# Eclectic-Sheep/sheeprl

Measured on NVIDIA H100. Metric: Dreamer-V3 train-steps/sec (S, bs16 seq64 horizon15, 64x64x3 obs), higher is better.
Workload: dtype f32

## Files before the change

sheeprl_b200/csrc/rssm_scan.cu:

```cuda
#include "b200rl.h"
#include "common.cuh"

namespace {

constexpr int SCAN_G = 128;
constexpr int SCAN_NT = 512;
constexpr int SCAN_NW = SCAN_NT / 32;
constexpr int MAXB = 16;
constexpr int MAXRPU = 8;
constexpr int KS_MAX = 8;
constexpr int CLS_SLICES = 8;

typedef unsigned long long u64;

__host__ __device__ inline int r4(int x) { return (x + 3) / 4 * 4; }
__host__ __device__ inline int imax(int a, int b) { return a > b ? a : b; }
__host__ __device__ inline int imin(int a, int b) { return a < b ? a : b; }

__host__ __device__ inline int owned_groups(int width, int cta) {
  const int groups = (width + 3) / 4;
  return (groups > cta) ? (groups - cta + SCAN_G - 1) / SCAN_G : 0;
}
__host__ __device__ inline int owned_cols(int width, int cta) {
  int n = 0;
  for (int gi = cta; gi * 4 < width; gi += SCAN_G) n += (width - gi * 4 < 4) ? width - gi * 4 : 4;
  return n;
}

struct Workspace {
  int* error;
  long long* prof;
  u64* ll;
  int* zidx;
  float* ln_stats;
};

struct LLGeo {
  size_t z, x, sx, s, h, r, a, b, c, d, sb, sc, sd, total;
};

__host__ __device__ inline LLGeo make_ll(int S, int Dx, int R, int Dr, int Z) {
  LLGeo g;
  size_t o = 0;
  g.z = o; o += 2 * (size_t)MAXB * S;
  g.x = o; o += 2 * (size_t)MAXB * Dx;
  g.sx = o; o += 2 * (size_t)MAXB * SCAN_G * 2;
  g.s = o; o += 2 * (size_t)MAXB * SCAN_G * 2;
  g.h = o; o += 2 * (size_t)MAXB * R;
  g.r = o; o += 2 * (size_t)MAXB * Dr;
  g.a = o; o += 2 * (size_t)MAXB * Z;
  g.b = o; o += 2 * (size_t)MAXB * Dr;
  g.c = o; o += 2 * (size_t)MAXB * 3 * R;
  g.d = o; o += 2 * (size_t)MAXB * Dx;
  g.sb = o; o += 2 * (size_t)MAXB * SCAN_G * 2;
  g.sc = o; o += 2 * (size_t)MAXB * SCAN_G * 2;
  g.sd = o; o += 2 * (size_t)MAXB * SCAN_G * 2;
  g.total = o;
  return g;
}

constexpr size_t WS_HEADER = 256, WS_PROF = 2 * 32 * sizeof(long long);

__host__ __device__ inline size_t ws_ll_bytes(int S, int D, int Dx, int R, int Dr) {
  return make_ll(S, Dx, R, Dr, S * D).total * sizeof(u64);
}
__host__ __device__ inline size_t ws_bytes(int T, int B, int S, int D, int Dx, int R, int Dr) {
  return WS_HEADER + WS_PROF + ws_ll_bytes(S, D, Dx, R, Dr) + sizeof(int) * (size_t)T * B * S +
         sizeof(float) * 3 * (size_t)T * B * 2 + 256;
}
// ... 33 lines not shown
  bool dead;
  __device__ __forceinline__ void init(int* e) { error = e; polls = 0; t0 = 0; dead = false; }
  __device__ __forceinline__ bool fail() {
    if (dead) return true;
    if ((++polls & 255u) == 0u) {
      if (t0 == 0) t0 = clock64();
      if (clock64() - t0 > 4000000000LL) { atomicExch(error, 1); dead = true; }
      else if (*(volatile int*)error != 0) dead = true;
    }
    return dead;
  }
};

__device__ __forceinline__ float ll_wait(const u64* p, unsigned tag, Spin& sp) {
  u64 v = ll_load(p);
  while ((unsigned)(v >> 32) != tag) {
    if (sp.fail()) break;
    v = ll_load(p);
  }
  return __uint_as_float((unsigned)v);
}

template <int LL_UNROLL>
__device__ __noinline__ void ll_recv(float* dst, int ds, const u64* src, int ss, int rows, int n, unsigned tag, int tid, Spin& sp) {
  const int half = n >> 1;
  int rg = 0, kp = tid, nrg = 1, kstep = SCAN_NT;
  if (half < SCAN_NT) { rg = tid / half; kp = tid - rg * half; nrg = SCAN_NT / half; kstep = half; if (rg >= nrg) return; }
  for (int k = 2 * kp; k < n; k += 2 * kstep) {
    for (int r0 = rg; r0 < rows; r0 += nrg * LL_UNROLL) {
      u64 a[LL_UNROLL], b[LL_UNROLL];
#pragma unroll
      for (int u = 0; u < LL_UNROLL; ++u)
        if (r0 + u * nrg < rows) ll_load2(src + (size_t)(r0 + u * nrg) * ss + k, a[u], b[u]);
      for (;;) {
        bool stale = false;
#pragma unroll
        for (int u = 0; u < LL_UNROLL; ++u)
          if (r0 + u * nrg < rows && ((unsigned)(a[u] >> 32) != tag || (unsigned)(b[u] >> 32) != tag)) stale = true;
        if (!stale || sp.fail()) break;
#pragma unroll
        for (int u = 0; u < LL_UNROLL; ++u)
          if (r0 + u * nrg < rows && ((unsigned)(a[u] >> 32) != tag || (unsigned)(b[u] >> 32) != tag))
            ll_load2(src + (size_t)(r0 + u * nrg) * ss + k, a[u], b[u]);
      }
#pragma unroll
      for (int u = 0; u < LL_UNROLL; ++u)
        if (r0 + u * nrg < rows)
          *reinterpret_cast<float2*>(dst + (r0 + u * nrg) * ds + k) =
              make_float2(__uint_as_float((unsigned)a[u]), __uint_as_float((unsigned)b[u]));
    }
  }
}

struct Slot {
  int b, cj, col;
  bool ok;
};
__device__ __forceinline__ Slot make_slot(int e, int per_row, int B, int cta, int width) {
  Slot s;
  s.b = per_row > 0 ? e / per_row : 0;
  s.cj = e - s.b * per_row;
  s.col = (cta + (s.cj >> 2) * SCAN_G) * 4 + (s.cj & 3);
  s.ok = per_row > 0 && s.b < B && s.col < width;
  return s;
}

__device__ __forceinline__ float fsilu(float x) { return __fdividef(x, 1.f + __expf(-x)); }

__device__ __forceinline__ void mma_tf32(float (&d)[4], const unsigned (&a)[4], unsigned b0, unsigned b1) {
  asm volatile("mma.sync.aligned.m16n8k8.row.col.f32.tf32.tf32.f32 {%0,%1,%2,%3}, {%4,%5,%6,%7}, {%8,%9}, {%0,%1,%2,%3};"
               : "+f"(d[0]), "+f"(d[1]), "+f"(d[2]), "+f"(d[3])
               : "r"(a[0]), "r"(a[1]), "r"(a[2]), "r"(a[3]), "r"(b0), "r"(b1));
}
__device__ __forceinline__ unsigned tf32_hi(float x) { return __float_as_uint(x) & 0xffffe000u; }
// ... 24 lines not shown
    }
    {
      const unsigned ah[4] = {tf32_hi(va.z), tf32_hi(vb.z), tf32_hi(va.w), tf32_hi(vb.w)};
      const unsigned al[4] = {tf32_lo(va.z), tf32_lo(vb.z), tf32_lo(va.w), tf32_lo(vb.w)};
      const unsigned bh0 = tf32_hi(vw.z), bh1 = tf32_hi(vw.w), bl0 = tf32_lo(vw.z), bl1 = tf32_lo(vw.w);
      mma_tf32(dx, ah, bl0, bl1);
      mma_tf32(dy, al, bh0, bh1);
      mma_tf32(d, ah, bh0, bh1);
    }
  }
#pragma unroll
  for (int i = 0; i < 4; ++i) d[i] += dx[i] + dy[i];
  const int c = 2 * t;
  if (c < nvalid) {
    part[(size_t)g * ldp + c0 + c] = d[0];
    part[(size_t)(g + 8) * ldp + c0 + c] = d[2];
  }
  if (c + 1 < nvalid) {
    part[(size_t)g * ldp + c0 + c + 1] = d[1];
    part[(size_t)(g + 8) * ldp + c0 + c + 1] = d[3];
  }
}

__device__ __noinline__ int product(const float* X, int xs, const float* wbase, int wst, int ngroups, int K, int B,
                                       float* PART, int ldp, int cbase, int tid) {
  if (ngroups <= 0) return 0;
  const int lane = tid & 31, wid = tid >> 5;
  const int ncols = ngroups * 4, ntiles = (ncols + 7) >> 3, Kp = r4(K);
  int ks = imin(KS_MAX, imax(1, SCAN_NW / ntiles));
  const int kchunk = ((Kp + ks - 1) / ks + 15) / 16 * 16;
  ks = (Kp + kchunk - 1) / kchunk;
  for (int item = wid; item < ntiles * ks; item += SCAN_NW) {
    const int sl = item / ntiles, tile = item - sl * ntiles;
    const int k0 = sl * kchunk, k1 = imin(Kp, k0 + kchunk);
    mma_item(X, xs, B, wbase + (size_t)tile * 8 * wst, wst, imin(8, ncols - tile * 8), k0, k1,
             PART + (size_t)sl * MAXB * ldp, ldp, cbase + tile * 8, lane);
  }
  return ks;
}

__device__ __forceinline__ float part_sum(const float* PART, int ldp, int ks, int b, int c) {
  float v = 0.f;
  for (int s = 0; s < ks; ++s) v += PART[((size_t)s * MAXB + b) * ldp + c];
  return v;
}

__device__ __noinline__ void class_product(const float* X, int xs, const float* W, int wst, int D, int Kp, int nr, float* PART,
                                              int tid) {
  const int lane = tid & 31, wid = tid >> 5, g = lane >> 2, t = lane & 3;
  const int sl = wid % CLS_SLICES, half = wid / CLS_SLICES;
  const int kc = ((Kp + CLS_SLICES - 1) / CLS_SLICES + 15) / 16 * 16;
  const int k0 = sl * kc, k1 = imin(Kp, k0 + kc);
  const int n0 = half * 16;
  if (n0 >= D) return;
  const bool r_ok = g < nr, n_ok0 = n0 + g < D, n_ok1 = n0 + 8 + g < D;
  const float* xa = X + (size_t)g * xs;
  const float* w0 = W + (size_t)(n0 + g) * wst;
  const float* w1 = W + (size_t)(n0 + 8 + g) * wst;
  float d0[4] = {0.f, 0.f, 0.f, 0.f}, d1[4] = {0.f, 0.f, 0.f, 0.f};
  float e0[4] = {0.f, 0.f, 0.f, 0.f}, e1[4] = {0.f, 0.f, 0.f, 0.f};
  for (int kb = k0; kb < k1; kb += 16) {
    const int k = kb + 4 * t;
    const bool k_ok = k < k1;
    float4 va = make_float4(0.f, 0.f, 0.f, 0.f), v0 = va, v1 = va;
    if (r_ok && k_ok) va = *reinterpret_cast<const float4*>(xa + k);
    if (n_ok0 && k_ok) v0 = *reinterpret_cast<const float4*>(w0 + k);
    if (n_ok1 && k_ok) v1 = *reinterpret_cast<const float4*>(w1 + k);
    {
      const unsigned ah[4] = {tf32_hi(va.x), 0u, tf32_hi(va.y), 0u}, al[4] = {tf32_lo(va.x), 0u, tf32_lo(va.y), 0u};
      mma_tf32(e0, ah, tf32_lo(v0.x), tf32_lo(v0.y)); mma_tf32(e1, ah, tf32_lo(v1.x), tf32_lo(v1.y));
// ... 94 lines not shown
  const int S = FIX ? 32 : a.S, D = FIX ? 32 : a.D, Z = S * D, R = FIX ? 512 : a.R, Dx = FIX ? 512 : a.Dx, Dr = FIX ? 512 : a.Dr;
  const int NB = T * B;
  const GeoF g = make_geo_f(Dims{B, S, D, R, Dx, Dr, a.A}, cta);
  const Workspace ws = carve(a.workspace, T, B, S, D, Dx, R, Dr);
  const LLGeo L = make_ll(S, Dx, R, Dr, Z);
  float* Wg = sm + g.oWg;
  float* Wr1 = sm + g.oWr1;
  float* W2 = sm + g.oW2;
  float* Xh = sm + g.oXh;
  float* Xx = sm + g.oXx;
  float* PART = sm + g.oPart;
  float* ACC = sm + g.oAcc;
  float* Win = sm + g.oWin;
  float* X0 = sm + g.oX0;
  float* H0 = sm + g.oPar;
  float* LNXG = H0 + g.sR;
  float* LNXB = LNXG + g.sDx;
  float* LNRG = LNXB + g.sDx;
  float* LNRB = LNRG + g.sDr;
  float* misc = sm + g.oMisc;
  int* z0idx = (int*)(sm + g.oInt);
  int* zall = z0idx + 64;
  int* nctab = zall + MAXB * 64;
  int* nxtab = nctab + SCAN_G;
  const int ldp = g.ldp, xxs = imax(g.sDx, g.sDr);
  const bool sampler = g.unit_g >= 0;
  __shared__ long long sprof[32];
  const bool prof_on = (cta < 2) && tid == 0;
  long long* prof = sprof;
  if (tid < 32) sprof[tid] = 0;
  long long tlast = prof_on ? clock64() : 0;
  Spin sp;
  sp.init(ws.error);

  for (int e = tid; e < g.total; e += SCAN_NT) sm[e] = 0.f;
  __syncthreads();
  for (int gi = 0; gi < g.ngh; ++gi)
    for (int part = 0; part < 3; ++part) {
      float* dst = Wg + (size_t)(gi * 3 + part) * 4 * g.wgst;
      const float* Wp = a.W_g + (size_t)part * R * (R + Dx);
      load_rows4(dst, g.wgst, 0, Wp, R + Dx, (cta + gi * SCAN_G) * 4, R, 0, R, g.sR, tid);
      load_rows4(dst, g.wgst, g.sR, Wp, R + Dx, (cta + gi * SCAN_G) * 4, R, R, Dx, g.sDx, tid);
    }
  for (int gi = 0; gi < g.ngr; ++gi)
    load_rows4(Wr1 + (size_t)gi * 4 * g.sR, g.sR, 0, a.W_r1, a.ld_wr1, (cta + gi * SCAN_G) * 4, Dr, 0, R, g.sR, tid);
  if (sampler)
    for (int e = tid; e < D * Dr; e += SCAN_NT) {
      const int d = e / Dr, k = e - d * Dr;
      W2[d * g.w2st + k] = a.W_r2[((size_t)g.unit_g * D + d) * Dr + k];
    }
  for (int k = tid; k < R; k += SCAN_NT) H0[k] = a.h0[k];
  for (int k = tid; k < Dx; k += SCAN_NT) { LNXG[k] = a.lnx_g[k]; LNXB[k] = a.lnx_b[k]; }
  for (int k = tid; k < Dr; k += SCAN_NT) { LNRG[k] = a.lnr_g[k]; LNRB[k] = a.lnr_b[k]; }
  for (int c = tid; c < SCAN_G; c += SCAN_NT) { nctab[c] = owned_cols(R, c); nxtab[c] = owned_cols(Dx, c); }
  for (int gi = 0; gi < g.ngx; ++gi)
    load_rows4(Win + (size_t)gi * 4 * g.kin, g.kin, 0, a.W_in, Z + A, (cta + gi * SCAN_G) * 4, Dx, 0, Z + A, g.kin, tid);
  if (wid == 0) {
    for (int gq = 0; gq < S; ++gq) {
      int best = 0;
      for (int d = lane; d < D; d += 32)
        if (a.z0[gq * D + d] > 0.5f) best = d;
#pragma unroll
      for (int o = 16; o > 0; o >>= 1) best = max(best, __shfl_xor_sync(0xffffffffu, best, o));
      if (lane == 0) z0idx[gq] = best;
    }
  }
  __syncthreads();
  for (int cj = tid; cj < g.ngx * 4; cj += SCAN_NT) {
    float acc = 0.f;
    for (int gq = 0; gq < S; ++gq) acc += Win[(size_t)cj * g.kin + gq * D + z0idx[gq]];
    X0[cj] = acc;
  }
  if (sampler)
    for (int e = tid; e < g.unit_nr * D; e += SCAN_NT) {
      const int b = g.unit_r0 + e / D, d = e % D;
      a.z_in[(size_t)b * Z + g.unit_g * D + d] = a.first[b] * ((z0idx[g.unit_g] == d) ? 1.f : 0.f);
    }
  const int nh4 = g.ngh * 4, nh12 = g.ngh * 12, nr4 = g.ngr * 4, nx4 = g.ngx * 4;
  const Slot sH = make_slot(tid, nh4, B, cta, R);
  const Slot sX = make_slot(tid, nx4, B, cta, Dx);
  const int nxcol = owned_cols(Dx, cta);
  const Slot sR_ = make_slot(tid, nr4, B, cta, Dr);
  const int pb = nh12 > 0 ? tid / nh12 : 0, pc = tid - pb * nh12;
  const int pcol = (cta + (pc / 12) * SCAN_G) * 4 + (pc & 3), ppart = (pc % 12) >> 2;
  const bool pok = nh12 > 0 && pb < B && pcol < R;
  float lg_g[3] = {0.f, 0.f, 0.f}, lg_b[3] = {0.f, 0.f, 0.f};
  if (sH.ok)
#pragma unroll
    for (int part = 0; part < 3; ++part) { lg_g[part] = a.lng_g[part * R + sH.col]; lg_b[part] = a.lng_b[part * R + sH.col]; }
  const int ncol3 = 3 * owned_cols(R, cta);
  const float bias2 = (sampler && lane < D) ? a.b_r2[g.unit_g * D + lane] : 0.f;
  float first_next = (tid < B) ? a.first[tid] : 0.f;
  __syncthreads();
  prof_mark(prof, 0, tlast, prof_on);

  for (int t = 0; t < T; ++t) {
    const size_t row0 = (size_t)t * B;
    const int par = t & 1;
    const unsigned tag = (unsigned)t + 1u;
    if (tid < MAXB) misc[tid] = first_next;
    if (tid < MAXB) first_next = (tid < B && t + 1 < T) ? a.first[row0 + B + tid] : 0.f;
    const float pe_pref = sR_.ok ? a.pe[(row0 + sR_.b) * Dr + sR_.col] : 0.f;
    float noise_pref = 1.f, fnext = 0.f;
    if (sampler && wid < g.unit_nr) {
      if (lane < D) noise_pref = a.noise[(row0 + g.unit_r0 + wid) * Z + (size_t)g.unit_g * D + lane];
      if (t + 1 < T) fnext = a.first[row0 + B + g.unit_r0 + wid];
    }
    __syncthreads();
    const float* fl = misc;

    if (t > 0)
      for (int e = tid; e < B * S; e += SCAN_NT) {
        const int b = e / S, gq = e - b * S;
        zall[b * 64 + gq] = (int)__float_as_uint(ll_wait(ws.ll + L.z + ((size_t)(par ^ 1) * MAXB + b) * S + gq, (unsigned)t, sp));
      }
    __syncthreads();
    prof_mark(prof, 2, tlast, prof_on);
    for (int b = wid; b < B; b += SCAN_NW) {
      const float f = fl[b];
      float rowv[4] = {0.f, 0.f, 0.f, 0.f};
      float rs = 0.f;
      int rcnt = 0;
      for (int c0 = 0; c0 < nx4; c0 += 4) {
        const int cj = c0 + (lane >> 3), part = lane & 7;
        const int col = (cta + (cj >> 2) * SCAN_G) * 4 + (cj & 3);
        const bool okc = cj < nx4 && col < Dx;
        float acc = 0.f;
        if (okc && t > 0 && f != 1.f) {
          const float* wrow = Win + (size_t)cj * g.kin;
          const int gper = (S + 7) >> 3, g_lo = part * gper, g_hi = imin(S, g_lo + gper);
          for (int gq = g_lo; gq < g_hi; ++gq) acc += wrow[gq * D + zall[b * 64 + gq]];
        }
        acc += __shfl_xor_sync(0xffffffffu, acc, 4);
        acc += __shfl_xor_sync(0xffffffffu, acc, 2);
        acc += __shfl_xor_sync(0xffffffffu, acc, 1);
        if (okc && part == 0) {
          float aa = 0.f;
          for (int qq = 0; qq < A; ++qq) aa = fmaf(a.actions[(row0 + b) * A + qq], Win[(size_t)cj * g.kin + Z + qq], aa);
          const float xv = (1.f - f) * (acc + aa) + f * X0[cj];
          ll_store(ws.ll + L.x + ((size_t)par * MAXB + b) * Dx + col, xv, tag);
          a.x_pre[(row0 + b) * Dx + col] = xv;
          rowv[c0 >> 2] = xv;
          rs += xv;
          ++rcnt;
        }
      }
      rs = warp_sum(rs);
      const float mean = nxcol > 0 ? rs / (float)nxcol : 0.f;
      float m2 = 0.f;
      for (int i = 0; i < 4; ++i)
        if (i < rcnt) { const float d = rowv[i] - mean; m2 = fmaf(d, d, m2); }
      m2 = warp_sum(m2);
      if (lane == 0) ll_store2(ws.ll + L.sx + (((size_t)par * MAXB + b) * SCAN_G + cta) * 2, mean, m2, tag);
    }
    if (cta == (t % SCAN_G))
      for (int e = tid; e < B * A; e += SCAN_NT) a.a_in[row0 * A + e] = (1.f - fl[e / A]) * a.actions[row0 * A + e];
    prof_mark(prof, 3, tlast, prof_on);

    for (int b = 0; b < B; ++b) {
      const float f = fl[b];
      if (f != 0.f || t == 0)
        for (int k = tid; k < R; k += SCAN_NT) Xh[b * g.sR + k] = (1.f - f) * ((t > 0) ? Xh[b * g.sR + k] : 0.f) + f * H0[k];
    }
    __syncthreads();
    prof_mark(prof, 12, tlast, prof_on);
    const int ksh = product(Xh, g.sR, Wg, g.wgst, g.ngh * 3, R, B, PART, ldp, 0, tid);
    prof_mark(prof, 1, tlast, prof_on);
    __syncthreads();
    const float acch = pok ? part_sum(PART, ldp, ksh, pb, pc) : 0.f;
    const float hin = sH.ok ? Xh[sH.b * g.sR + sH.col] : 0.f;
    prof_mark(prof, 13, tlast, prof_on);

    ll_recv<8>(Xx, xxs, ws.ll + L.x + (size_t)par * MAXB * Dx, Dx, B, Dx, tag, tid, sp);
    for (int b = wid; b < B; b += SCAN_NW) {
      float pm[SCAN_G / 32], pq[SCAN_G / 32];
      u64 x[SCAN_G / 32], y[SCAN_G / 32];
#pragma unroll
      for (int i = 0; i < SCAN_G / 32; ++i)
        ll_load2(ws.ll + L.sx + (((size_t)par * MAXB + b) * SCAN_G + lane + 32 * i) * 2, x[i], y[i]);
      for (;;) {
        bool stale = false;
#pragma unroll
        for (int i = 0; i < SCAN_G / 32; ++i)
          if ((unsigned)(x[i] >> 32) != tag || (unsigned)(y[i] >> 32) != tag) stale = true;
        if (!stale || sp.fail()) break;
#pragma unroll
        for (int i = 0; i < SCAN_G / 32; ++i)
          if ((unsigned)(x[i] >> 32) != tag || (unsigned)(y[i] >> 32) != tag)
            ll_load2(ws.ll + L.sx + (((size_t)par * MAXB + b) * SCAN_G + lane + 32 * i) * 2, x[i], y[i]);
      }
#pragma unroll
      for (int i = 0; i < SCAN_G / 32; ++i) {
        pm[i] = __uint_as_float((unsigned)x[i]);
        pq[i] = __uint_as_float((unsigned)y[i]);
      }
      float sm_ = 0.f;
#pragma unroll
      for (int i = 0; i < SCAN_G / 32; ++i) sm_ += (float)nxtab[lane + 32 * i] * pm[i];
      const float mean = warp_sum(sm_) / (float)Dx;
      float m2 = 0.f;
#pragma unroll
      for (int i = 0; i < SCAN_G / 32; ++i) {
        const float d = pm[i] - mean;
        m2 += pq[i] + (float)nxtab[lane + 32 * i] * d * d;
      }
      m2 = warp_sum(m2);
      if (lane == 0) {
        const float rstd = rsqrtf(m2 / (float)Dx + a.eps);
        misc[16 + b] = mean;
        misc[32 + b] = rstd;
        if (cta == ((t + 1) % SCAN_G)) {
          ws.ln_stats[((size_t)0 * NB + row0 + b) * 2] = mean;
          ws.ln_stats[((size_t)0 * NB + row0 + b) * 2 + 1] = rstd;
        }
      }
    }
    __syncthreads();
    for (int k = tid; k < Dx; k += SCAN_NT) {
      const float gk = LNXG[k], bk = LNXB[k];
      for (int b = 0; b < B; ++b)
        Xx[b * xxs + k] = fsilu((Xx[b * xxs + k] - misc[16 + b]) * misc[32 + b] * gk + bk);
    }
    __syncthreads();
    if (sX.ok) a.x_act[(row0 + sX.b) * Dx + sX.col] = Xx[sX.b * xxs + sX.col];
    prof_mark(prof, 4, tlast, prof_on);
    const int ksx = product(Xx, xxs, Wg + g.sR, g.wgst, g.ngh * 3, Dx, B, PART, ldp, 0, tid);
    __syncthreads();
    float gpre = 0.f;
    if (pok) {
      gpre = acch + part_sum(PART, ldp, ksx, pb, pc);
      ACC[pb * ldp + pc] = gpre;
    }
    __syncthreads();
    for (int b = wid; b < B; b += SCAN_NW) {
      float s = 0.f;
      for (int c = lane; c < nh12; c += 32)
        if ((cta + (c / 12) * SCAN_G) * 4 + (c & 3) < R) s += ACC[b * ldp + c];
      s = warp_sum(s);
      const float mean = ncol3 > 0 ? s / (float)ncol3 : 0.f;
      float m2 = 0.f;
      for (int c = lane; c < nh12; c += 32)
        if ((cta + (c / 12) * SCAN_G) * 4 + (c & 3) < R) { const float d = ACC[b * ldp + c] - mean; m2 = fmaf(d, d, m2); }
      m2 = warp_sum(m2);
      if (lane == 0) ll_store2(ws.ll + L.s + (((size_t)par * MAXB + b) * SCAN_G + cta) * 2, mean, m2, tag);
    }
    if (pok) a.g_pre[(row0 + pb) * 3 * R + ppart * R + pcol] = gpre;
    prof_mark(prof, 5, tlast, prof_on);

    for (int b0 = wid; b0 < B; b0 += 2 * SCAN_NW) {
      u64 x[2][SCAN_G / 32], y[2][SCAN_G / 32];
#pragma unroll
      for (int rr = 0; rr < 2; ++rr) {
        const int b = b0 + rr * SCAN_NW;
        if (b < B)
#pragma unroll
          for (int i = 0; i < SCAN_G / 32; ++i)
            ll_load2(ws.ll + L.s + (((size_t)par * MAXB + b) * SCAN_G + lane + 32 * i) * 2, x[rr][i], y[rr][i]);
      }
#pragma unroll
      for (int rr = 0; rr < 2; ++rr) {
        const int b = b0 + rr * SCAN_NW;
        if (b >= B) continue;
        float pm[SCAN_G / 32], pq[SCAN_G / 32];
        for (;;) {
          bool stale = false;
#pragma unroll
          for (int i = 0; i < SCAN_G / 32; ++i)
            if ((unsigned)(x[rr][i] >> 32) != tag || (unsigned)(y[rr][i] >> 32) != tag) stale = true;
          if (!stale || sp.fail()) break;
#pragma unroll
          for (int i = 0; i < SCAN_G / 32; ++i)
// ... 169 lines not shown
    g.unit_r0 = sp * g.rpu;
    g.unit_nr = imin(g.rpu, a.B - g.unit_r0);
    if (g.unit_nr > 0) g.unit_g = cta % a.S; else g.unit_nr = 0;
  }
  const int mh = owned_groups(a.R, 0), mx = owned_groups(a.Dx, 0), mr = owned_groups(a.Dr, 0);
  g.ldp = imax(imax((mh + mx) * 4, mr * 4), 4);
  int o = 0;
  g.oW2 = o;   o += mr * 4 * g.sZ;
  g.oW1 = o;   o += mh * 4 * g.sDr;
  g.oWg = o;   o += (mh + mx) * 4 * g.wgst;
  g.oWin = o;  o += a.D * g.winst;
  g.oX = o;    o += MAXB * g.xw;
  g.oPart = o; o += imax(KS_MAX * MAXB * g.ldp, CLS_SLICES * MAXRPU * 32);
  g.oAcc = o;  o += MAXB * g.ldp;
  g.oSt = o;   o += 2 * MAXB * imax(imax(mh * 12, mx * 4), imax(mr * 4, 4));
  g.oDhc = o;  o += MAXB * imax(mh * 4, 4);
  g.oDh0 = o;  o += imax(mh * 4, 4);
  g.oWs = o;   o += mh * 4 + (mh + mx) * 4 + 32;
  g.oMisc = o; o += 16 * MAXB + 64;
  g.total = o;
  return g;
}

__device__ __noinline__ void recv_row_sums(const u64* base, int par, int r0, int nr, unsigned tag, float inv, float* out1,
                                              float* out2, int tid, Spin& sp) {
  const int lane = tid & 31, wid = tid >> 5;
  for (int bb0 = wid; bb0 < nr; bb0 += 2 * SCAN_NW) {
    u64 x[2][SCAN_G / 32], y[2][SCAN_G / 32];
#pragma unroll
    for (int rr = 0; rr < 2; ++rr) {
      const int bb = bb0 + rr * SCAN_NW;
      if (bb < nr)
#pragma unroll
        for (int i = 0; i < SCAN_G / 32; ++i)
          ll_load2(base + (((size_t)par * MAXB + r0 + bb) * SCAN_G + lane + 32 * i) * 2, x[rr][i], y[rr][i]);
    }
#pragma unroll
    for (int rr = 0; rr < 2; ++rr) {
      const int bb = bb0 + rr * SCAN_NW;
      if (bb >= nr) continue;
      const int b = r0 + bb;
      float v0 = 0.f, v1 = 0.f;
      for (;;) {
        bool stale = false;
#pragma unroll
        for (int i = 0; i < SCAN_G / 32; ++i)
          if ((unsigned)(x[rr][i] >> 32) != tag || (unsigned)(y[rr][i] >> 32) != tag) stale = true;
        if (!stale || sp.fail()) break;
#pragma unroll
        for (int i = 0; i < SCAN_G / 32; ++i)
          if ((unsigned)(x[rr][i] >> 32) != tag || (unsigned)(y[rr][i] >> 32) != tag)
            ll_load2(base + (((size_t)par * MAXB + b) * SCAN_G + lane + 32 * i) * 2, x[rr][i], y[rr][i]);
      }
#pragma unroll
      for (int i = 0; i < SCAN_G / 32; ++i) {
        v0 += __uint_as_float((unsigned)x[rr][i]);
        v1 += __uint_as_float((unsigned)y[rr][i]);
      }
      v0 = warp_sum(v0); v1 = warp_sum(v1);
      if (lane == 0) { out1[b] = v0 * inv; out2[b] = v1 * inv; }
    }
  }
}

__device__ __noinline__ void send_row_sums(const float* ST, int ncols, int B, u64* base, int par, int cta, unsigned tag, int tid) {
  const int lane = tid & 31, wid = tid >> 5;
  for (int b = wid; b < B; b += SCAN_NW) {
    float s1 = 0.f, s2 = 0.f;
    for (int c = lane; c < ncols; c += 32) { s1 += ST[(b * ncols + c) * 2]; s2 += ST[(b * ncols + c) * 2 + 1]; }
    s1 = warp_sum(s1); s2 = warp_sum(s2);
    if (lane == 0) ll_store2(base + (((size_t)par * MAXB + b) * SCAN_G + cta) * 2, s1, s2, tag);
  }
}

template <bool FIX>
__global__ void __launch_bounds__(SCAN_NT, 1)
rssm_scan_bwd_kernel(const b200rl_rssm_scan_args a, const b200rl_rssm_scan_grads q) {
  extern __shared__ __align__(16) float sm[];
  const int tid = threadIdx.x, lane = tid & 31, wid = tid >> 5;
  const int cta = blockIdx.x;
  const int T = a.T, B = a.B;
  const int S = FIX ? 32 : a.S, D = FIX ? 32 : a.D, Z = S * D, R = FIX ? 512 : a.R, Dx = FIX ? 512 : a.Dx, Dr = FIX ? 512 : a.Dr;
  const int KG = R + Dx, KIN = Z + a.A, NB = T * B;
  const GeoB g = make_geo_b(Dims{B, S, D, R, Dx, Dr, a.A}, cta);
  const Workspace ws = carve(a.workspace, T, B, S, D, Dx, R, Dr);
  const LLGeo L = make_ll(S, Dx, R, Dr, Z);
  const int mh = owned_groups(R, 0), mx = owned_groups(Dx, 0);
  float* W2T = sm + g.oW2;
// ... 104 lines not shown
      p_qgh = q.q_g[(row0 + sH.b) * KG + sH.col];
#pragma unroll
      for (int part = 0; part < 3; ++part) {
        p_gl[part] = a.g_ln[(row0 + sH.b) * 3 * R + part * R + sH.col];
        p_gp[part] = a.g_pre[(row0 + sH.b) * 3 * R + part * R + sH.col];
      }
    }
    const float p_xp = sX.ok ? a.x_pre[(row0 + sX.b) * Dx + sX.col] : 0.f;
    const float p_qgx = sX.ok ? q.q_g[(row0 + sX.b) * KG + R + sX.col] : 0.f;
    float u_dl = 0.f, u_dmix = 0.f, u_raw = -INFINITY, u_qx = 0.f;
    if (unit && wid < g.unit_nr && lane < D) {
      const size_t o = (row0 + g.unit_r0 + wid) * Z + (size_t)g.unit_g * D + lane;
      u_dl = q.d_latent[(row0 + g.unit_r0 + wid) * a.ld_lat + (size_t)g.unit_g * D + lane];
      u_dmix = q.d_post_mix[o];
      u_raw = a.post_raw[o];
      if (!last) u_qx = q.q_x[(row0 + B + g.unit_r0 + wid) * Z + (size_t)g.unit_g * D + lane];
    }
    __syncthreads();
    const float* fl = misc;

    if (unit) {
      const int gq = g.unit_g, nr = g.unit_nr, rb = g.unit_r0;
      if (!last) {
        ll_recv<4>(X, xw, ws.ll + L.d + ((size_t)(par ^ 1) * MAXB + rb) * Dx, Dx, nr, Dx, (unsigned)bt, tid, sp);
        recv_row_sums(ws.ll + L.sd, par ^ 1, rb, nr, (unsigned)bt, 1.f / (float)Dx, S1, S2, tid, sp);
        __syncthreads();
        prof_mark(prof, 17, tlast, prof_on);
        class_product(X, xw, WinU, g.winst, D, g.sDx, nr, PART, tid);
        __syncthreads();
      }
      if (wid < nr) {
        const int bb = wid, b = rb + bb;
        const bool on = lane < D;
        float dz = u_dl;
        if (!last) {
          float p1 = 0.f;
          for (int s2 = 0; s2 < CLS_SLICES; ++s2) p1 += PART[((size_t)s2 * MAXRPU + bb) * 32 + lane];
          if (on) {
            const float mu = LNX1[b * 2], rstd = LNX1[b * 2 + 1];
            const float p2 = rstd * (u_qx - mu * wsi);
            dz += (1.f - fl[16 + b]) * rstd * (p1 - S1[b] * wsi - S2[b] * p2);
          }
        }
        const float mx_ = warp_max(u_raw);
        const float ex = on ? expf(u_raw - mx_) : 0.f;
        const float sft = ex / warp_sum(ex);
        float gg = u_dmix;
        if (a.unimix > 0.f) {
// ... 23 lines not shown
    __syncthreads();
    prof_mark(prof, 19, tlast, prof_on);
    const int ks2 = product(X, xw, W2T, g.sZ, g.ngr, Z, B, PART, ldp, 0, tid);
    __syncthreads();
    float dact_r = 0.f;
    if (sR_.ok) {
      dact_r = part_sum(PART, ldp, ks2, sR_.b, sR_.cj);
      const float xh = (p_rp - LNS[(2 * MAXB + sR_.b) * 2]) * LNS[(2 * MAXB + sR_.b) * 2 + 1];
      const float ln = xh * gam_r + bet_r;
      const float sg = sigmoidf_(ln);
      const float dxh = dact_r * sg * (1.f + ln * (1.f - sg)) * gam_r;
      ll_store(ws.ll + L.b + ((size_t)par * MAXB + sR_.b) * Dr + sR_.col, dxh, tag);
      ST[(sR_.b * nr4 + sR_.cj) * 2] = dxh;
      ST[(sR_.b * nr4 + sR_.cj) * 2 + 1] = dxh * xh;
    } else if (tid < B * nr4) {
      ST[tid * 2] = 0.f; ST[tid * 2 + 1] = 0.f;
    }
    __syncthreads();
    send_row_sums(ST, nr4, B, ws.ll + L.sb, par, cta, tag, tid);
    if (sR_.ok) q.d_rp_act[(row0 + sR_.b) * Dr + sR_.col] = dact_r;
    prof_mark(prof, 20, tlast, prof_on);

    __syncthreads();
    ll_recv<4>(X, xw, ws.ll + L.b + (size_t)par * MAXB * Dr, Dr, B, Dr, tag, tid, sp);
    recv_row_sums(ws.ll + L.sb, par, 0, B, tag, 1.f / (float)Dr, S1, S2, tid, sp);
    __syncthreads();
    prof_mark(prof, 21, tlast, prof_on);
    const int ks1 = product(X, xw, W1T, g.sDr, g.ngh, Dr, B, PART, ldp, 0, tid);
    __syncthreads();
    float dhin_gate = 0.f, dgl[3] = {0.f, 0.f, 0.f};
    if (sH.ok) {
      const int b = sH.b;
      const float mur = LNS[(2 * MAXB + b) * 2], rstdr = LNS[(2 * MAXB + b) * 2 + 1];
      const float mug = LNS[(1 * MAXB + b) * 2], rstdg = LNS[(1 * MAXB + b) * 2 + 1];
      const float p1 = part_sum(PART, ldp, ks1, b, sH.cj);
      const float p2 = rstdr * (p_qr - mur * ws1);
      float dh = p_dlh + rstdr * (p1 - S1[b] * ws1 - S2[b] * p2);
      if (!last) dh += DHC[b * nh4 + sH.cj];
      const float r = sigmoidf_(p_gl[0]), cnd = tanhf(r * p_gl[1]), u = sigmoidf_(p_gl[2] - 1.f);
      const float du = dh * (cnd - p_hin);
      const float drc = dh * u * (1.f - cnd * cnd);
      dgl[0] = drc * p_gl[1] * r * (1.f - r);
      dgl[1] = drc * r;
      dgl[2] = du * u * (1.f - u);
      dhin_gate = dh * (1.f - u);
#pragma unroll
      for (int part = 0; part < 3; ++part) {
        const float xh = (p_gp[part] - mug) * rstdg;
// ... 6 lines not shown
      const int b = tid / imax(nh4, 1), cj = tid - b * nh4;
#pragma unroll
      for (int part = 0; part < 3; ++part) {
        ST[(b * (3 * nh4) + part * nh4 + cj) * 2] = 0.f;
        ST[(b * (3 * nh4) + part * nh4 + cj) * 2 + 1] = 0.f;
      }
    }
    __syncthreads();
    send_row_sums(ST, 3 * nh4, B, ws.ll + L.sc, par, cta, tag, tid);
    if (sH.ok)
#pragma unroll
      for (int part = 0; part < 3; ++part) q.d_g_ln[(row0 + sH.b) * 3 * R + part * R + sH.col] = dgl[part];
    prof_mark(prof, 22, tlast, prof_on);

    __syncthreads();
    for (int part = 0; part < 2; ++part)
      ll_recv<4>(X + part * g.sR, xw, ws.ll + L.c + (size_t)par * MAXB * 3 * R + (size_t)part * R, 3 * R, B, R, tag, tid, sp);
    __syncthreads();
    const int ksa = product(X, xw, WgT, g.wgst, g.ngh + g.ngx, 2 * g.sR, B, PART, ldp, 0, tid);
    __syncthreads();
    float acc_h = sH.ok ? part_sum(PART, ldp, ksa, sH.b, sH.cj) : 0.f;
    float acc_x = sX.ok ? part_sum(PART, ldp, ksa, sX.b, nh4 + sX.cj) : 0.f;
    __syncthreads();
    ll_recv<4>(X, xw, ws.ll + L.c + (size_t)par * MAXB * 3 * R + (size_t)2 * R, 3 * R, B, R, tag, tid, sp);
    recv_row_sums(ws.ll + L.sc, par, 0, B, tag, 1.f / (float)(3 * R), S1, S2, tid, sp);
    __syncthreads();
    const int ksb = product(X, xw, WgT + 2 * g.sR, g.wgst, g.ngh + g.ngx, R, B, PART, ldp, 0, tid);
    __syncthreads();
    prof_mark(prof, 23, tlast, prof_on);
    float dact_x = 0.f;
    if (sX.ok) {
      const int b = sX.b;
      acc_x += part_sum(PART, ldp, ksb, b, nh4 + sX.cj);
      const float mug = LNS[(1 * MAXB + b) * 2], rstdg = LNS[(1 * MAXB + b) * 2 + 1];
      const float mux = LNS[(0 * MAXB + b) * 2], rstdx = LNS[(0 * MAXB + b) * 2 + 1];
      const float p2 = rstdg * (p_qgx - mug * wsgx);
      dact_x = rstdg * (acc_x - S1[b] * wsgx - S2[b] * p2);
      const float xh = (p_xp - mux) * rstdx;
      const float ln = xh * gam_x + bet_x;
      const float sg = sigmoidf_(ln);
      const float dxh = dact_x * sg * (1.f + ln * (1.f - sg)) * gam_x;
      ll_store(ws.ll + L.d + ((size_t)par * MAXB + b) * Dx + sX.col, dxh, tag);
      ST[(b * nx4 + sX.cj) * 2] = dxh;
      ST[(b * nx4 + sX.cj) * 2 + 1] = dxh * xh;
    } else if (tid < B * nx4) {
      ST[tid * 2] = 0.f; ST[tid * 2 + 1] = 0.f;
    }
    float dhin_f = 0.f;
// ... 75 lines not shown
  GeoG g;
  g.ngh = owned_groups(R, cta);
  g.sR = r4(R);
  const int mh = owned_groups(R, 0);
  g.ldp = backward ? mh * 4 : mh * 12;
  for (g.pw = backward ? 3 : 1;; g.pw = 1) {
    int o = 0;
    g.oW = o;    o += mh * 12 * g.sR;
    g.oX = o;    o += MAXB * g.pw * g.sR;
    g.oPart = o; o += KS_MAX * MAXB * g.ldp;
    g.oAcc = o;  o += MAXB * g.ldp;
    g.oSt = o;   o += backward ? 2 * MAXB * mh * 12 : 0;
    g.oDhc = o;  o += backward ? MAXB * mh * 4 : 0;
    g.oPar = o;  o += backward ? mh * 4 : g.sR;
    g.oLn = o;   o += mh * 24;
    g.oMisc = o; o += 96;
    g.oTab = o;  o += SCAN_G;
    g.total = o;
    if (g.pw == 1 || sizeof(float) * (size_t)o <= 227 * 1024) break;
  }
  return g;
}

__device__ __noinline__ void merge_row_stats(const u64* base, unsigned tag, const int* cnt, float n, float eps, int lane,
                                                Spin& sp, float& mean, float& rstd) {
  u64 x[SCAN_G / 32], y[SCAN_G / 32];
#pragma unroll
  for (int i = 0; i < SCAN_G / 32; ++i) ll_load2(base + (lane + 32 * i) * 2, x[i], y[i]);
  for (;;) {
    bool stale = false;
#pragma unroll
    for (int i = 0; i < SCAN_G / 32; ++i)
      if ((unsigned)(x[i] >> 32) != tag || (unsigned)(y[i] >> 32) != tag) stale = true;
    if (!stale || sp.fail()) break;
#pragma unroll
    for (int i = 0; i < SCAN_G / 32; ++i)
      if ((unsigned)(x[i] >> 32) != tag || (unsigned)(y[i] >> 32) != tag) ll_load2(base + (lane + 32 * i) * 2, x[i], y[i]);
  }
  float sm_ = 0.f;
#pragma unroll
  for (int i = 0; i < SCAN_G / 32; ++i) sm_ += (float)cnt[lane + 32 * i] * __uint_as_float((unsigned)x[i]);
  mean = warp_sum(sm_) / n;
  float m2 = 0.f;
#pragma unroll
  for (int i = 0; i < SCAN_G / 32; ++i) {
    const float d = __uint_as_float((unsigned)x[i]) - mean;
    m2 += __uint_as_float((unsigned)y[i]) + (float)cnt[lane + 32 * i] * d * d;
// ... 201 lines not shown
      for (int part = 0; part < 3; ++part) {
        const float xh = (p_gp[part] - mug) * rstdg;
        const float dxh = dgl[part] * LNP[part * nh4 + sH.cj];
        ll_store(ll + L.c + ((size_t)par * MAXB + b) * 3 * R + (size_t)part * R + sH.col, dxh, tag);
        ST[(b * (3 * nh4) + part * nh4 + sH.cj) * 2] = dxh;
        ST[(b * (3 * nh4) + part * nh4 + sH.cj) * 2 + 1] = dxh * xh;
      }
    } else if (tid < B * nh4) {
      const int b = tid / imax(nh4, 1), cj = tid - b * nh4;
#pragma unroll
      for (int part = 0; part < 3; ++part) {
        ST[(b * (3 * nh4) + part * nh4 + cj) * 2] = 0.f;
        ST[(b * (3 * nh4) + part * nh4 + cj) * 2 + 1] = 0.f;
      }
    }
    __syncthreads();
    send_row_sums(ST, 3 * nh4, B, ll + L.sc, par, cta, tag, tid);
    if (sH.ok)
#pragma unroll
      for (int part = 0; part < 3; ++part) q.d_g_ln[(row0 + sH.b) * 3 * R + (size_t)part * R + sH.col] = dgl[part];

    float acc_h = 0.f;
    for (int p0 = 0; p0 < 3; p0 += g.pw) {
      for (int part = p0; part < p0 + g.pw; ++part)
        ll_recv<4>(X + (part - p0) * g.sR, xw, ll + L.c + (size_t)par * MAXB * 3 * R + (size_t)part * R, 3 * R, B, R, tag, tid, sp);
      if (p0 == 0) recv_row_sums(ll + L.sc, par, 0, B, tag, 1.f / (float)(3 * R), S1, S2, tid, sp);
      __syncthreads();
      const int ks = product(X, xw, WgT + p0 * g.sR, wgst, g.ngh, g.pw * g.sR, B, PART, ldp, 0, tid);
      __syncthreads();
      if (sH.ok) acc_h += part_sum(PART, ldp, ks, sH.b, sH.cj);
      __syncthreads();
    }
    float dhin_f = 0.f;
    if (sH.ok) {
      const int b = sH.b;
      const float mug = LNS[b * 2], rstdg = LNS[b * 2 + 1];
      const float wsgh = WSG[sH.cj];
      const float p2 = rstdg * (p_qg - mug * wsgh);
      const float dhin = dhin_gate + rstdg * (acc_h - S1[b] * wsgh - S2[b] * p2);
      DHC[b * nh4 + sH.cj] = (1.f - fl[b]) * dhin;
      dhin_f = fl[b] * dhin;
    }
    if (sH.ok) ACC[sH.b * ldp + sH.cj] = dhin_f;
    __syncthreads();
    if (tid < nh4)
      for (int b = 0; b < B; ++b)
        if (fl[b] != 0.f) dh0_acc += ACC[b * ldp + tid];
    __syncthreads();
    if (sp.dead) break;
// ... 103 lines not shown
```

Baseline: 60.20.

## Fuse row-sum polling into ll_recv and compute input LN stats locally

Row-sum receives now poll inside ll_recv, interleaved with the data receive, instead of running as a separate recv_row_sums pass. In the forward scan each CTA no longer publishes per-CTA mean/M2 partials over the LL buffer (sx region removed). Each CTA instead computes the LayerNorm mean and variance itself from the full received x rows, one warp per row. Several device helpers change from noinline to forceinline. This trades extra cross-CTA messages and a wait phase for redundant local reduction work and higher register pressure.

```diff
diff --git a/sheeprl_b200/csrc/rssm_scan.cu b/sheeprl_b200/csrc/rssm_scan.cu
--- a/sheeprl_b200/csrc/rssm_scan.cu
+++ b/sheeprl_b200/csrc/rssm_scan.cu
@@ -36,7 +36,7 @@
 };
 
 struct LLGeo {
-  size_t z, x, sx, s, h, r, a, b, c, d, sb, sc, sd, total;
+  size_t z, x, s, h, r, a, b, c, d, sb, sc, sd, total;
 };
 
 __host__ __device__ inline LLGeo make_ll(int S, int Dx, int R, int Dr, int Z) {
@@ -44,7 +44,6 @@
   size_t o = 0;
   g.z = o; o += 2 * (size_t)MAXB * S;
   g.x = o; o += 2 * (size_t)MAXB * Dx;
-  g.sx = o; o += 2 * (size_t)MAXB * SCAN_G * 2;
   g.s = o; o += 2 * (size_t)MAXB * SCAN_G * 2;
   g.h = o; o += 2 * (size_t)MAXB * R;
   g.r = o; o += 2 * (size_t)MAXB * Dr;
@@ -124,34 +123,66 @@
 }
 
 template <int LL_UNROLL>
-__device__ __noinline__ void ll_recv(float* dst, int ds, const u64* src, int ss, int rows, int n, unsigned tag, int tid, Spin& sp) {
+__device__ __forceinline__ void ll_recv(float* dst, int ds, const u64* src, int ss, int rows, int n, unsigned tag, int tid, Spin& sp,
+                                     const u64* sums = nullptr, int sr0 = 0, float inv = 0.f, float* out1 = nullptr,
+                                     float* out2 = nullptr) {
+  static_assert(MAXB <= SCAN_NW, "one warp per row of the row sums");
+  const int lane = tid & 31, wid = tid >> 5;
+  const bool has_s = sums != nullptr && wid < rows;
+  const u64* sp_row = has_s ? sums + ((size_t)(sr0 + wid) * SCAN_G + lane) * 2 : nullptr;
+  u64 sx[SCAN_G / 32], sy[SCAN_G / 32];
+  bool s_stale = has_s;
+  if (has_s)
+#pragma unroll
+    for (int i = 0; i < SCAN_G / 32; ++i) ll_load2(sp_row + 64 * i, sx[i], sy[i]);
+  auto poll_sums = [&]() {
+    if (!s_stale) return false;
+    bool st = false;
+#pragma unroll
+    for (int i = 0; i < SCAN_G / 32; ++i)
+      if ((unsigned)(sx[i] >> 32) != tag || (unsigned)(sy[i] >> 32) != tag) { st = true; ll_load2(sp_row + 64 * i, sx[i], sy[i]); }
+    s_stale = st;
+    return st;
+  };
   const int half = n >> 1;
   int rg = 0, kp = tid, nrg = 1, kstep = SCAN_NT;
-  if (half < SCAN_NT) { rg = tid / half; kp = tid - rg * half; nrg = SCAN_NT / half; kstep = half; if (rg >= nrg) return; }
-  for (int k = 2 * kp; k < n; k += 2 * kstep) {
-    for (int r0 = rg; r0 < rows; r0 += nrg * LL_UNROLL) {
-      u64 a[LL_UNROLL], b[LL_UNROLL];
-#pragma unroll
-      for (int u = 0; u < LL_UNROLL; ++u)
-        if (r0 + u * nrg < rows) ll_load2(src + (size_t)(r0 + u * nrg) * ss + k, a[u], b[u]);
-      for (;;) {
-        bool stale = false;
+  if (half < SCAN_NT) { rg = tid / half; kp = tid - rg * half; nrg = SCAN_NT / half; kstep = half; }
+  if (rg < nrg)
+    for (int k = 2 * kp; k < n; k += 2 * kstep) {
+      for (int r0 = rg; r0 < rows; r0 += nrg * LL_UNROLL) {
+        u64 a[LL_UNROLL], b[LL_UNROLL];
 #pragma unroll
         for (int u = 0; u < LL_UNROLL; ++u)
-          if (r0 + u * nrg < rows && ((unsigned)(a[u] >> 32) != tag || (unsigned)(b[u] >> 32) != tag)) stale = true;
-        if (!stale || sp.fail()) break;
+          if (r0 + u * nrg < rows) ll_load2(src + (size_t)(r0 + u * nrg) * ss + k, a[u], b[u]);
+        for (;;) {
+          bool stale = false;
+#pragma unroll
+          for (int u = 0; u < LL_UNROLL; ++u)
+            if (r0 + u * nrg < rows && ((unsigned)(a[u] >> 32) != tag || (unsigned)(b[u] >> 32) != tag)) stale = true;
+          if (!stale || sp.fail()) break;
+#pragma unroll
+          for (int u = 0; u < LL_UNROLL; ++u)
+            if (r0 + u * nrg < rows && ((unsigned)(a[u] >> 32) != tag || (unsigned)(b[u] >> 32) != tag))
+              ll_load2(src + (size_t)(r0 + u * nrg) * ss + k, a[u], b[u]);
+          poll_sums();
+        }
 #pragma unroll
         for (int u = 0; u < LL_UNROLL; ++u)
-          if (r0 + u * nrg < rows && ((unsigned)(a[u] >> 32) != tag || (unsigned)(b[u] >> 32) != tag))
-            ll_load2(src + (size_t)(r0 + u * nrg) * ss + k, a[u], b[u]);
-      }
-#pragma unroll
-      for (int u = 0; u < LL_UNROLL; ++u)
-        if (r0 + u * nrg < rows)
-          *reinterpret_cast<float2*>(dst + (r0 + u * nrg) * ds + k) =
-              make_float2(__uint_as_float((unsigned)a[u]), __uint_as_float((unsigned)b[u]));
-    }
-  }
+          if (r0 + u * nrg < rows)
+            *reinterpret_cast<float2*>(dst + (r0 + u * nrg) * ds + k) =
+                make_float2(__uint_as_float((unsigned)a[u]), __uint_as_float((unsigned)b[u]));
+      }
+    }
+  if (!has_s) return;
+  while (poll_sums() && !sp.fail()) {}
+  float v0 = 0.f, v1 = 0.f;
+#pragma unroll
+  for (int i = 0; i < SCAN_G / 32; ++i) {
+    v0 += __uint_as_float((unsigned)sx[i]);
+    v1 += __uint_as_float((unsigned)sy[i]);
+  }
+  v0 = warp_sum(v0); v1 = warp_sum(v1);
+  if (lane == 0) { out1[sr0 + wid] = v0 * inv; out2[sr0 + wid] = v1 * inv; }
 }
 
 struct Slot {
@@ -222,7 +253,7 @@
   }
 }
 
-__device__ __noinline__ int product(const float* X, int xs, const float* wbase, int wst, int ngroups, int K, int B,
+__device__ __forceinline__ int product(const float* X, int xs, const float* wbase, int wst, int ngroups, int K, int B,
                                        float* PART, int ldp, int cbase, int tid) {
   if (ngroups <= 0) return 0;
   const int lane = tid & 31, wid = tid >> 5;
@@ -245,7 +276,7 @@
   return v;
 }
 
-__device__ __noinline__ void class_product(const float* X, int xs, const float* W, int wst, int D, int Kp, int nr, float* PART,
+__device__ __forceinline__ void class_product(const float* X, int xs, const float* W, int wst, int D, int Kp, int nr, float* PART,
                                               int tid) {
   const int lane = tid & 31, wid = tid >> 5, g = lane >> 2, t = lane & 3;
   const int sl = wid % CLS_SLICES, half = wid / CLS_SLICES;
@@ -386,7 +417,6 @@
   int* z0idx = (int*)(sm + g.oInt);
   int* zall = z0idx + 64;
   int* nctab = zall + MAXB * 64;
-  int* nxtab = nctab + SCAN_G;
   const int ldp = g.ldp, xxs = imax(g.sDx, g.sDr);
   const bool sampler = g.unit_g >= 0;
   __shared__ long long sprof[32];
@@ -416,7 +446,7 @@
   for (int k = tid; k < R; k += SCAN_NT) H0[k] = a.h0[k];
   for (int k = tid; k < Dx; k += SCAN_NT) { LNXG[k] = a.lnx_g[k]; LNXB[k] = a.lnx_b[k]; }
   for (int k = tid; k < Dr; k += SCAN_NT) { LNRG[k] = a.lnr_g[k]; LNRB[k] = a.lnr_b[k]; }
-  for (int c = tid; c < SCAN_G; c += SCAN_NT) { nctab[c] = owned_cols(R, c); nxtab[c] = owned_cols(Dx, c); }
+  for (int c = tid; c < SCAN_G; c += SCAN_NT) nctab[c] = owned_cols(R, c);
   for (int gi = 0; gi < g.ngx; ++gi)
     load_rows4(Win + (size_t)gi * 4 * g.kin, g.kin, 0, a.W_in, Z + A, (cta + gi * SCAN_G) * 4, Dx, 0, Z + A, g.kin, tid);
   if (wid == 0) {
@@ -443,15 +473,10 @@
   const int nh4 = g.ngh * 4, nh12 = g.ngh * 12, nr4 = g.ngr * 4, nx4 = g.ngx * 4;
   const Slot sH = make_slot(tid, nh4, B, cta, R);
   const Slot sX = make_slot(tid, nx4, B, cta, Dx);
-  const int nxcol = owned_cols(Dx, cta);
   const Slot sR_ = make_slot(tid, nr4, B, cta, Dr);
   const int pb = nh12 > 0 ? tid / nh12 : 0, pc = tid - pb * nh12;
   const int pcol = (cta + (pc / 12) * SCAN_G) * 4 + (pc & 3), ppart = (pc % 12) >> 2;
   const bool pok = nh12 > 0 && pb < B && pcol < R;
-  float lg_g[3] = {0.f, 0.f, 0.f}, lg_b[3] = {0.f, 0.f, 0.f};
-  if (sH.ok)
-#pragma unroll
-    for (int part = 0; part < 3; ++part) { lg_g[part] = a.lng_g[part * R + sH.col]; lg_b[part] = a.lng_b[part * R + sH.col]; }
   const int ncol3 = 3 * owned_cols(R, cta);
   const float bias2 = (sampler && lane < D) ? a.b_r2[g.unit_g * D + lane] : 0.f;
   float first_next = (tid < B) ? a.first[tid] : 0.f;
@@ -482,9 +507,6 @@
     prof_mark(prof, 2, tlast, prof_on);
     for (int b = wid; b < B; b += SCAN_NW) {
       const float f = fl[b];
-      float rowv[4] = {0.f, 0.f, 0.f, 0.f};
-      float rs = 0.f;
-      int rcnt = 0;
       for (int c0 = 0; c0 < nx4; c0 += 4) {
         const int cj = c0 + (lane >> 3), part = lane & 7;
         const int col = (cta + (cj >> 2) * SCAN_G) * 4 + (cj & 3);
@@ -504,18 +526,8 @@
           const float xv = (1.f - f) * (acc + aa) + f * X0[cj];
           ll_store(ws.ll + L.x + ((size_t)par * MAXB + b) * Dx + col, xv, tag);
           a.x_pre[(row0 + b) * Dx + col] = xv;
-          rowv[c0 >> 2] = xv;
-          rs += xv;
-          ++rcnt;
         }
       }
-      rs = warp_sum(rs);
-      const float mean = nxcol > 0 ? rs / (float)nxcol : 0.f;
-      float m2 = 0.f;
-      for (int i = 0; i < 4; ++i)
-        if (i < rcnt) { const float d = rowv[i] - mean; m2 = fmaf(d, d, m2); }
-      m2 = warp_sum(m2);
-      if (lane == 0) ll_store2(ws.ll + L.sx + (((size_t)par * MAXB + b) * SCAN_G + cta) * 2, mean, m2, tag);
     }
     if (cta == (t % SCAN_G))
       for (int e = tid; e < B * A; e += SCAN_NT) a.a_in[row0 * A + e] = (1.f - fl[e / A]) * a.actions[row0 * A + e];
@@ -536,54 +548,20 @@
     prof_mark(prof, 13, tlast, prof_on);
 
     ll_recv<8>(Xx, xxs, ws.ll + L.x + (size_t)par * MAXB * Dx, Dx, B, Dx, tag, tid, sp);
+    __syncthreads();
     for (int b = wid; b < B; b += SCAN_NW) {
-      float pm[SCAN_G / 32], pq[SCAN_G / 32];
-      u64 x[SCAN_G / 32], y[SCAN_G / 32];
-#pragma unroll
-      for (int i = 0; i < SCAN_G / 32; ++i)
-        ll_load2(ws.ll + L.sx + (((size_t)par * MAXB + b) * SCAN_G + lane + 32 * i) * 2, x[i], y[i]);
-      for (;;) {
-        bool stale = false;
-#pragma unroll
-        for (int i = 0; i < SCAN_G / 32; ++i)
-          if ((unsigned)(x[i] >> 32) != tag || (unsigned)(y[i] >> 32) != tag) stale = true;
-        if (!stale || sp.fail()) break;
-#pragma unroll
-        for (int i = 0; i < SCAN_G / 32; ++i)
-          if ((unsigned)(x[i] >> 32) != tag || (unsigned)(y[i] >> 32) != tag)
-            ll_load2(ws.ll + L.sx + (((size_t)par * MAXB + b) * SCAN_G + lane + 32 * i) * 2, x[i], y[i]);
-      }
-#pragma unroll
-      for (int i = 0; i < SCAN_G / 32; ++i) {
-        pm[i] = __uint_as_float((unsigned)x[i]);
-        pq[i] = __uint_as_float((unsigned)y[i]);
-      }
-      float sm_ = 0.f;
-#pragma unroll
-      for (int i = 0; i < SCAN_G / 32; ++i) sm_ += (float)nxtab[lane + 32 * i] * pm[i];
-      const float mean = warp_sum(sm_) / (float)Dx;
+      float* xr = Xx + b * xxs;
+      float s = 0.f;
+      for (int k = lane; k < Dx; k += 32) s += xr[k];
+      const float mean = warp_sum(s) / (float)Dx;
       float m2 = 0.f;
-#pragma unroll
-      for (int i = 0; i < SCAN_G / 32; ++i) {
-        const float d = pm[i] - mean;
-        m2 += pq[i] + (float)nxtab[lane + 32 * i] * d * d;
-      }
-      m2 = warp_sum(m2);
-      if (lane == 0) {
-        const float rstd = rsqrtf(m2 / (float)Dx + a.eps);
-        misc[16 + b] = mean;
-        misc[32 + b] = rstd;
-        if (cta == ((t + 1) % SCAN_G)) {
-          ws.ln_stats[((size_t)0 * NB + row0 + b) * 2] = mean;
-          ws.ln_stats[((size_t)0 * NB + row0 + b) * 2 + 1] = rstd;
-        }
-      }
-    }
-    __syncthreads();
-    for (int k = tid; k < Dx; k += SCAN_NT) {
-      const float gk = LNXG[k], bk = LNXB[k];
-      for (int b = 0; b < B; ++b)
-        Xx[b * xxs + k] = fsilu((Xx[b * xxs + k] - misc[16 + b]) * misc[32 + b] * gk + bk);
+      for (int k = lane; k < Dx; k += 32) { const float d = xr[k] - mean; m2 = fmaf(d, d, m2); }
+      const float rstd = rsqrtf(warp_sum(m2) / (float)Dx + a.eps);
+      for (int k = lane; k < Dx; k += 32) xr[k] = fsilu((xr[k] - mean) * rstd * LNXG[k] + LNXB[k]);
+      if (lane == 0 && cta == ((t + 1) % SCAN_G)) {
+        ws.ln_stats[((size_t)0 * NB + row0 + b) * 2] = mean;
+        ws.ln_stats[((size_t)0 * NB + row0 + b) * 2 + 1] = rstd;
+      }
     }
     __syncthreads();
     if (sX.ok) a.x_act[(row0 + sX.b) * Dx + sX.col] = Xx[sX.b * xxs + sX.col];
@@ -611,6 +589,10 @@
     if (pok) a.g_pre[(row0 + pb) * 3 * R + ppart * R + pcol] = gpre;
     prof_mark(prof, 5, tlast, prof_on);
 
+    float lg_g[3] = {0.f, 0.f, 0.f}, lg_b[3] = {0.f, 0.f, 0.f};
+    if (sH.ok)
+#pragma unroll
+      for (int part = 0; part < 3; ++part) { lg_g[part] = a.lng_g[part * R + sH.col]; lg_b[part] = a.lng_b[part * R + sH.col]; }
     for (int b0 = wid; b0 < B; b0 += 2 * SCAN_NW) {
       u64 x[2][SCAN_G / 32], y[2][SCAN_G / 32];
 #pragma unroll
@@ -826,48 +808,7 @@
   return g;
 }
 
-__device__ __noinline__ void recv_row_sums(const u64* base, int par, int r0, int nr, unsigned tag, float inv, float* out1,
-                                              float* out2, int tid, Spin& sp) {
-  const int lane = tid & 31, wid = tid >> 5;
-  for (int bb0 = wid; bb0 < nr; bb0 += 2 * SCAN_NW) {
-    u64 x[2][SCAN_G / 32], y[2][SCAN_G / 32];
-#pragma unroll
-    for (int rr = 0; rr < 2; ++rr) {
-      const int bb = bb0 + rr * SCAN_NW;
-      if (bb < nr)
-#pragma unroll
-        for (int i = 0; i < SCAN_G / 32; ++i)
-          ll_load2(base + (((size_t)par * MAXB + r0 + bb) * SCAN_G + lane + 32 * i) * 2, x[rr][i], y[rr][i]);
-    }
-#pragma unroll
-    for (int rr = 0; rr < 2; ++rr) {
-      const int bb = bb0 + rr * SCAN_NW;
-      if (bb >= nr) continue;
-      const int b = r0 + bb;
-      float v0 = 0.f, v1 = 0.f;
-      for (;;) {
-        bool stale = false;
-#pragma unroll
-        for (int i = 0; i < SCAN_G / 32; ++i)
-          if ((unsigned)(x[rr][i] >> 32) != tag || (unsigned)(y[rr][i] >> 32) != tag) stale = true;
-        if (!stale || sp.fail()) break;
-#pragma unroll
-        for (int i = 0; i < SCAN_G / 32; ++i)
-          if ((unsigned)(x[rr][i] >> 32) != tag || (unsigned)(y[rr][i] >> 32) != tag)
-            ll_load2(base + (((size_t)par * MAXB + b) * SCAN_G + lane + 32 * i) * 2, x[rr][i], y[rr][i]);
-      }
-#pragma unroll
-      for (int i = 0; i < SCAN_G / 32; ++i) {
-        v0 += __uint_as_float((unsigned)x[rr][i]);
-        v1 += __uint_as_float((unsigned)y[rr][i]);
-      }
-      v0 = warp_sum(v0); v1 = warp_sum(v1);
-      if (lane == 0) { out1[b] = v0 * inv; out2[b] = v1 * inv; }
-    }
-  }
-}
-
-__device__ __noinline__ void send_row_sums(const float* ST, int ncols, int B, u64* base, int par, int cta, unsigned tag, int tid) {
+__device__ __forceinline__ void send_row_sums(const float* ST, int ncols, int B, u64* base, int par, int cta, unsigned tag, int tid) {
   const int lane = tid & 31, wid = tid >> 5;
   for (int b = wid; b < B; b += SCAN_NW) {
     float s1 = 0.f, s2 = 0.f;
@@ -1018,8 +959,8 @@
     if (unit) {
       const int gq = g.unit_g, nr = g.unit_nr, rb = g.unit_r0;
       if (!last) {
-        ll_recv<4>(X, xw, ws.ll + L.d + ((size_t)(par ^ 1) * MAXB + rb) * Dx, Dx, nr, Dx, (unsigned)bt, tid, sp);
-        recv_row_sums(ws.ll + L.sd, par ^ 1, rb, nr, (unsigned)bt, 1.f / (float)Dx, S1, S2, tid, sp);
+        ll_recv<4>(X, xw, ws.ll + L.d + ((size_t)(par ^ 1) * MAXB + rb) * Dx, Dx, nr, Dx, (unsigned)bt, tid, sp,
+                   ws.ll + L.sd + (size_t)(par ^ 1) * MAXB * SCAN_G * 2, rb, 1.f / (float)Dx, S1, S2);
         __syncthreads();
         prof_mark(prof, 17, tlast, prof_on);
         class_product(X, xw, WinU, g.winst, D, g.sDx, nr, PART, tid);
@@ -1089,8 +1030,8 @@
     prof_mark(prof, 20, tlast, prof_on);
 
     __syncthreads();
-    ll_recv<4>(X, xw, ws.ll + L.b + (size_t)par * MAXB * Dr, Dr, B, Dr, tag, tid, sp);
-    recv_row_sums(ws.ll + L.sb, par, 0, B, tag, 1.f / (float)Dr, S1, S2, tid, sp);
+    ll_recv<4>(X, xw, ws.ll + L.b + (size_t)par * MAXB * Dr, Dr, B, Dr, tag, tid, sp,
+               ws.ll + L.sb + (size_t)par * MAXB * SCAN_G * 2, 0, 1.f / (float)Dr, S1, S2);
     __syncthreads();
     prof_mark(prof, 21, tlast, prof_on);
     const int ks1 = product(X, xw, W1T, g.sDr, g.ngh, Dr, B, PART, ldp, 0, tid);
@@ -1143,8 +1084,8 @@
     float acc_h = sH.ok ? part_sum(PART, ldp, ksa, sH.b, sH.cj) : 0.f;
     float acc_x = sX.ok ? part_sum(PART, ldp, ksa, sX.b, nh4 + sX.cj) : 0.f;
     __syncthreads();
-    ll_recv<4>(X, xw, ws.ll + L.c + (size_t)par * MAXB * 3 * R + (size_t)2 * R, 3 * R, B, R, tag, tid, sp);
-    recv_row_sums(ws.ll + L.sc, par, 0, B, tag, 1.f / (float)(3 * R), S1, S2, tid, sp);
+    ll_recv<4>(X, xw, ws.ll + L.c + (size_t)par * MAXB * 3 * R + (size_t)2 * R, 3 * R, B, R, tag, tid, sp,
+               ws.ll + L.sc + (size_t)par * MAXB * SCAN_G * 2, 0, 1.f / (float)(3 * R), S1, S2);
     __syncthreads();
     const int ksb = product(X, xw, WgT + 2 * g.sR, g.wgst, g.ngh + g.ngx, R, B, PART, ldp, 0, tid);
     __syncthreads();
@@ -1266,7 +1207,7 @@
   return g;
 }
 
-__device__ __noinline__ void merge_row_stats(const u64* base, unsigned tag, const int* cnt, float n, float eps, int lane,
+__device__ __forceinline__ void merge_row_stats(const u64* base, unsigned tag, const int* cnt, float n, float eps, int lane,
                                                 Spin& sp, float& mean, float& rstd) {
   u64 x[SCAN_G / 32], y[SCAN_G / 32];
 #pragma unroll
@@ -1514,9 +1455,14 @@
 
     float acc_h = 0.f;
     for (int p0 = 0; p0 < 3; p0 += g.pw) {
-      for (int part = p0; part < p0 + g.pw; ++part)
-        ll_recv<4>(X + (part - p0) * g.sR, xw, ll + L.c + (size_t)par * MAXB * 3 * R + (size_t)part * R, 3 * R, B, R, tag, tid, sp);
-      if (p0 == 0) recv_row_sums(ll + L.sc, par, 0, B, tag, 1.f / (float)(3 * R), S1, S2, tid, sp);
+      for (int part = p0; part < p0 + g.pw; ++part) {
+        const u64* src = ll + L.c + (size_t)par * MAXB * 3 * R + (size_t)part * R;
+        if (part == g.pw - 1)
+          ll_recv<4>(X + (part - p0) * g.sR, xw, src, 3 * R, B, R, tag, tid, sp, ll + L.sc + (size_t)par * MAXB * SCAN_G * 2, 0,
+                     1.f / (float)(3 * R), S1, S2);
+        else
+          ll_recv<4>(X + (part - p0) * g.sR, xw, src, 3 * R, B, R, tag, tid, sp);
+      }
       __syncthreads();
       const int ks = product(X, xw, WgT + p0 * g.sR, wgst, g.ngh, g.pw * g.sR, B, PART, ldp, 0, tid);
       __syncthreads();
```

New measurement: 62.26, median of 6. +3.4%, better.
